# glgerard/MDBN

Measured on AMD Instinct MI355X. Metric: CD-k Gibbs steps/sec (samples/sec), GRBM 4096->1024 CD-1, higher is better.
Workload: dtype f32; 1 GPU; GRBM 4096->1024 CD-1, batch 512 per GPU, fp32, N(0,1) rows resident in HBM (BASELINE configs[1]); global_batch=512, k=1, n_data=32768, parallelism=dp1

## Files before the change

### mdbn_amd/csrc/mdbn_capi.hip

```cpp
#include <hip/hip_runtime.h>
#include "row_pool.h"
#include <dlfcn.h>
#include <algorithm>
#include <atomic>
#include <chrono>
#include <condition_variable>
#include <cstdint>
#include <deque>
#include <initializer_list>
#include <map>
#include <mutex>
#include <set>
#include <thread>
#include <cstdarg>
#include <cstdio>
#include <cstring>
#include <string>
#include <utility>
#include <vector>
#include "mdbn_kernels.h"
#include "mdbn_small.h"
#include "mdbn_thin.h"
#include "mdbn_gchain.h"
#include "mdbn_ais.h"
// ... 754 lines not shown
            EpiArgs e{};
            e.ld = ldh; e.bias = a->hbias; e.mean = keep ? nh : nullptr; e.mean_scale = -1.0f; e.gauss = 0;
            e.sample = (need_sample && keep) ? a->hs : nullptr; e.rng = key((uint32_t)(2 * t));
            e.mean_planes = pb.Pp + B * ldh; e.plane_stride = pb.pp;
            e.sample_plane = need_sample ? pb.hsp : nullptr;
            if (last) { e.colsum = ws.colPneg; e.colsum_kind = 0; }
            if (a->gauss) CHECK(run_affine_planes(ctx, a->comm_cus, pb.Xp + B * ldv, ldv, pb.px, 3, 0, Wp, V, H, Hlive, B, e, false, ws, s, nullptr));
            else CHECK(run_affine_planes(ctx, a->comm_cus, pb.vsp, ldv, B * ldv, 1, 0, Wp, V, H, Hlive, B, e, false, ws, s, nullptr));
            if (a->trace_h && need_sample)
                HIP_OK(hipMemcpyAsync(a->trace_h + (int64_t)t * B * ldh, a->hs, sizeof(float) * B * ldh, hipMemcpyDeviceToDevice, s));
        }
    }
    return MDBN_OK;
}

int planes_statistics(mdbn_ctx* ctx, hipStream_t s, const mdbn_cd_args* a, const Workspace& ws, const PlaneStep& pb, int n_cost,
                      const mdbn_update_args* upd, const mdbn_update_args* defer)
{
    const int64_t B = a->B, V = a->V, Hlive = a->H, ldv = V, ldh = a->ldh, H = ldh;
    const StatsView st(a->stats, V, ldv, ldh);
    const Plan sp = plan_stats(V, H, 2 * B, ldh, false);
    PlaneGemmArgs g{};
    g.A = pb.Xp; g.lda = ldv; g.pa = pb.px; g.ap = 3;
    g.B = pb.Pp; g.ldb = ldh; g.pb = pb.pp;
    g.M = (int)V; g.N = (int)H; g.K = (int)(2 * B);
    g.tiles_m = (int)(V / 128); g.tiles_n = (int)(H / 128); g.splitk = sp.splitk; g.kchunk = sp.kchunk;
    g.fin_enabled = 0;
    int bal = sp.splitk == 1 ? bal_blocks(ctx, a->comm_cus, (int64_t)g.tiles_m * g.tiles_n, 2 * B / 32) : 0;
    if (bal && ((int64_t)bal * 2 * 16384 > ws.slab_floats || V * ldh * 4 >= (int64_t)1 << 31)) bal = 0;
    const bool fuse_upd = !bal && upd != nullptr && g_opt_fused_update && sp.splitk == 1;
    auto set_gather_ahead = [&]() {
        if (g.upd.early && g_opt_gather_ahead && a->next_indexes && pb.Xother && !pb.keep) {
            const int nwg = g.tiles_m * g.tiles_n, nt = (int)(2 * B / 32);
            const int rpw = (int)((B + nwg - 1) / nwg), passes = (int)((ldv / 8 + 255) / 256);
            if (rpw * passes <= 4 && 16 / (nt >= 20 ? 1 : 2) + 4 + 1 <= nt - 3) {
                g.ga.src = a->data; g.ga.n_rows = a->n_data; g.ga.ld_src = ldv;
                g.ga.idx = a->next_indexes; g.ga.idx64 = a->index_is_64;
                g.ga.B = (int)B; g.ga.rpw = rpw; g.ga.passes = passes;
                g.ga.P = pb.Xother; g.ga.plane_stride = pb.px; g.ga.ld = ldv;
                if (a->ahead_done) *a->ahead_done = 1;
            }
        }
    };
    if (fuse_upd) {
        BiasUpd bu;
        fill_bias_upd(bu, *upd, Hlive);
        g.fused = 2;
        g.fin_enabled = 1;
        g.fin = make_fin_args(ws.colPpos, ws.colPneg, ws.colV, row_groups(B), ldh, ldv, ws.cost_partials, n_cost, st.s_h, st.s_v,
                              st.cost, &bu);
        fill_upd(g.upd, *upd, V, ldh, pb.Wp);
        g.upd.early = g_opt_early_w && upd->lambda_1 == 0.f && (upd->weightcost == 0.f || upd->W0 != nullptr) &&
                      2 * B / 32 >= 12 && g_opt_planes_mfma == 16 && !g_opt_bf16_inputs;
        set_gather_ahead();
        HIP_OK(timed_gemm_planes(LAY_MN, LAY_MN, g, s));
        return MDBN_OK;
    }
    if (sp.splitk == 1 && g_opt_fused_finalize) {
        g.fin_enabled = 1;
        g.fin = make_fin_args(ws.colPpos, ws.colPneg, ws.colV, row_groups(B), ldh, ldv, ws.cost_partials, n_cost, st.s_h, st.s_v,
                              st.cost, nullptr);
    } else {
        HIP_OK(launch_finalize_stats(ws.colPpos, ws.colPneg, ws.colV, row_groups(B), ldh, ldv, ws.cost_partials, n_cost, st.s_h,
                                     st.s_v, st.cost, nullptr, s));
    }
    g.fused = 0; g.ldc = ldh; g.slab_stride = V * ldh;
    if (defer) {
        const bool splitphase = g_opt_early_w && g_opt_planes_mfma == 16 && !g_opt_bf16_inputs && defer->phase == 3 &&
                                defer->lambda_1 == 0.f && (defer->weightcost == 0.f || defer->W0 != nullptr) &&
                                defer->stats != a->stats;
        const int64_t flat = bal ? (((V * ldh / 4 + bal - 1) / bal + 511) / 512) * 512 : 0;
        const bool inside = splitphase && (bal ? (flat <= 16 * 512 && (int64_t)g.tiles_m * g.tiles_n * (2 * B / 32) / bal >= 20)
                                               : (sp.splitk == 1 && 2 * B / 32 >= 20));
        g.upd.flat_per_wg = flat;
        if (inside) {
            fill_upd(g.upd, *defer, V, ldh, reinterpret_cast<unsigned short*>(defer->W_planes));
            g.upd.l1 = 0.f; g.upd.Sprev = defer->stats; g.upd.early = 2;
            const StatsView prev(const_cast<float*>(defer->stats), V, ldv, ldh);
            DeferredBias& d = g.db;
            d.on = 1; d.hb = defer->hbias; d.hbs = defer->hbias_speed; d.vb = defer->vbias; d.vbs = defer->vbias_speed;
            d.s_h = prev.s_h; d.s_v = prev.s_v; d.cost_sum = prev.cost; d.H = Hlive; d.V = V;
            d.lr = defer->lr; d.mu = defer->momentum; d.inv_rows = 1.0f / defer->n_rows;
            d.cost_scale = defer->cost_scale; d.cost_out = defer->cost_out;
            if (!bal) set_gather_ahead();
        } else {
            HIP_OK(launch_whole_update(*defer, s));
        }
    }
    if (bal) {
        g.xcd_group = 1;
        g.C = st.S; g.bal = bal; g.fused = 4; g.kchunk = (int)(2 * B); g.c_bytes = V * ldh * 4;
        g.scratch = ws.slabs;
        HIP_OK(timed_gemm_planes(LAY_MN, LAY_MN, g, s));
    } else if (sp.splitk == 1) {
        g.C = st.S;
        HIP_OK(timed_gemm_planes(LAY_MN, LAY_MN, g, s));
    } else {
        REQUIRE(sp.slab_floats(V, ldh) <= ws.slab_floats, "internal: statistic slabs exceed workspace");
        g.C = ws.slabs;
        HIP_OK(timed_gemm_planes(LAY_MN, LAY_MN, g, s));
        if (upd && g_opt_fused_update) {
            HIP_OK(launch_update(whole_rule(*upd), s, ws.slabs, sp.splitk, g.slab_stride, pb.Wp));
            return MDBN_OK;
        }
        HIP_OK(launch_sum_slabs(ws.slabs, sp.splitk, g.slab_stride, V * ldh, st.S, s));
    }
// ... 2044 lines not shown
```

### mdbn_amd/csrc/mdbn_kernels.h

```cpp
#pragma once
#include <hip/hip_runtime.h>
#include <stdint.h>
#include "philox.h"
#include "../../include/mdbn_hip.h"

namespace mdbn {

enum { LAY_K = 0, LAY_MN = 1 };

struct EpiArgs {
    const float* slabs;
    int64_t slab_stride;
    int nsplit;
    int rows, cols;
    int64_t ld;
    const float* bias;
    float* pre;
    float* mean;
    float* sample;
    float mean_scale;
    int gauss;
    const float* target;
    int64_t ld_target;
    const void* target_idx;
// ... 50 lines not shown
    const float* A;
    const float* B;
    float* C;
    int64_t lda, ldb, ldc;
    int64_t slab_stride;
    int M, N, K;
    int Nst;
    int kchunk;
    int splitk, tiles_m, tiles_n;
    int bn;
    int bk;
    int inner_m;
    int x6;
    int x6_pw;
    int cw;
    unsigned long long* stamps;
    int skinny;
    int mi;
    int ni;
    int fused;
    EpiArgs epi;
    UpdEpi upd;
    int fin_enabled;
    FinArgs fin;
};



struct GatherAhead {
    const float* src; int64_t n_rows, ld_src;
    const void* idx; int idx64;
    int B, rpw, passes;
    unsigned short* P; int64_t plane_stride, ld;
};

struct PlaneGemmArgs {
    const unsigned short* A; int64_t lda, pa;
    const unsigned short* B; int64_t ldb, pb;
    float* C; int64_t ldc, slab_stride;
    int M, N, K, kchunk, splitk, tiles_m, tiles_n;
    int ap;
    int ms;
    int bn;
    int fused;
    int slab_tail;
    unsigned long long* stamps;
    int bal;
    int xcd_group;
    float* scratch;
    int64_t c_bytes;
    EpiArgs epi;
    UpdEpi upd;
    int fin_enabled;
    FinArgs fin;
    GatherAhead ga;
    DeferredBias db;
};

__host__ __device__ inline int bal_first_unit(int w, int P, int64_t U) { return (int)(((int64_t)w * U) / P); }
__host__ __device__ inline int bal_block_of(int64_t u, int P, int64_t U) { return (int)(((u + 1) * P - 1) / U); }
__host__ __device__ inline int bal_rem_blocks(int tiles, int S, int P)
{
    const int64_t Ur = (int64_t)(tiles - (tiles / P) * P) * S;
    return Ur < P ? (int)Ur : P;
}
__host__ __device__ inline int bal_tile_slabs(int t, int tiles, int S, int P)
{
    const int Tf = (tiles / P) * P;
    if (t < Tf) return 1;
    const int64_t Ur = (int64_t)(tiles - Tf) * S, u0 = (int64_t)(t - Tf) * S;
    const int Pr = bal_rem_blocks(tiles, S, P);
    return bal_block_of(u0 + S - 1, Pr, Ur) - bal_block_of(u0, Pr, Ur) + 1;
}
hipError_t launch_gemm_planes(int la, int lb, const PlaneGemmArgs& g, hipStream_t s);
bool slab_tail_ok(const PlaneGemmArgs& g, int la, int lb);
hipError_t launch_gemm_planes_bal(int la, int lb, const PlaneGemmArgs& g, hipStream_t s);
int bal_max_segments(int tiles, int stages, int P);
int bal_segment_host(int tiles, int S, int P, int w, int k, int* tile, int* s0, int* s1, int* nseg, int* nt);
hipError_t launch_split_planes(const float* X, int64_t rows, int64_t ld, unsigned short* P, int64_t plane_stride, hipStream_t s);
hipError_t launch_gather_planes(const float* src, int64_t n_rows, int64_t cols_ld, int64_t ld_src, const void* idx, int idx64,
                                int64_t n_idx, float* dst, int64_t ld_dst, unsigned short* P, int64_t plane_stride, hipStream_t s);

int epilogue_blocks(int64_t rows, int64_t ld);
int epilogue_cw(int64_t rows, int64_t ld);
void set_epilogue_cw(int cw);
void set_epilogue_threads(int t);
inline int row_groups(int64_t B) { return (int)((B + 3) / 4); }

hipError_t launch_gemm(int la, int lb, const GemmArgs& g, hipStream_t s);
hipError_t launch_act_epilogue(const EpiArgs& e, hipStream_t s);
hipError_t launch_sum_slabs(const float* slabs, int nsplit, int64_t slab_stride, int64_t n,
                            float* out, hipStream_t s);
hipError_t launch_gather_slim(const float* src, int64_t n_rows, int64_t cols_ld, int64_t ld_src, const void* idx, int idx64,
                              int64_t n_idx, float* dst, int64_t ld_dst, int blocks, int threads, hipStream_t s);
hipError_t launch_gather(const float* src, int64_t n_rows, int64_t cols_ld, int64_t ld_src,
                         const void* idx, int idx64, int64_t n_idx, float* dst, int64_t ld_dst,
                         hipStream_t s);
hipError_t launch_colsum_groups(const float* X, const float* Y, int rows, int64_t ld, float* out, hipStream_t s);
FinArgs make_fin_args(const float* posP, const float* negP, const float* partV, int ngroups, int64_t ldh, int64_t ldv,
                      const float* cost_partials, int n_cost, float* s_h, float* s_v, float* cost,
                      const BiasUpd* bias_update);
hipError_t launch_finalize_stats(const float* posP, const float* negP, const float* partV, int ngroups,
                                 int64_t ldh, int64_t ldv, const float* cost_partials, int n_cost,
                                 float* s_h, float* s_v, float* cost, const BiasUpd* bias_update, hipStream_t s);
hipError_t launch_update(const mdbn_update_args& a, hipStream_t s, const float* slabs = nullptr, int nslab = 1,
                         int64_t slab_stride = 0, unsigned short* Wp = nullptr);
hipError_t launch_free_energy(const float* slabs, int nsplit, int64_t slab_stride, int64_t ldh, int H,
                              const float* hbias, const float* x, int64_t ldv, int V, const float* vbias,
                              int gauss, int64_t rows, float* out, hipStream_t s);
hipError_t launch_round_flip(const float* x, float* out, int64_t rows, int64_t cols, int64_t ld, int64_t flip_col, hipStream_t s);
hipError_t launch_pl_cost(const float* fe, const float* fe_flip, int64_t rows, float n_visible, float* out, hipStream_t s);
hipError_t launch_recon_cost(const float* pre, int64_t ldp, const float* tgt, int64_t ldt, int64_t rows, int64_t cols, int gauss,
                             float scale, float* partials, int n_partials, float* out, hipStream_t s);
hipError_t launch_tanh(float* x, int64_t rows, int64_t cols, int64_t ld, hipStream_t s);
hipError_t launch_count_nonfinite(const float* x, int64_t n, int* count, hipStream_t s);
hipError_t launch_narrow_bf16(const float* x, unsigned short* y, int64_t n, hipStream_t s);
hipError_t launch_widen_bf16(const unsigned short* y, float* x, int64_t n, hipStream_t s);
hipError_t launch_rng_fill(float* out, int64_t rows, int64_t cols, int64_t ld, const PhiloxKey& k,
                           int normal, hipStream_t s);

}
```

### mdbn_amd/csrc/mdbn_planes.hip

```cpp
#include <hip/hip_runtime.h>
#include <algorithm>
#include <stdint.h>
#include "mdbn_kernels.h"
#include "mdbn_device.h"

namespace mdbn {

typedef __bf16 pbf16x8 __attribute__((ext_vector_type(8)));
typedef short ps16x4 __attribute__((ext_vector_type(4)));
typedef short ps16x8 __attribute__((ext_vector_type(8)));
typedef float pf32x16 __attribute__((ext_vector_type(16)));
typedef float pf32x4 __attribute__((ext_vector_type(4)));
typedef unsigned int pu32x4b __attribute__((ext_vector_type(4)));

#ifndef PL_ARGS_EARLY
#define PL_ARGS_EARLY 1
#endif
constexpr int PL_PLANE = 8192, PL_STAGE = 6 * PL_PLANE, PL_NSTAGE = 3, PL_LW = 4;

__device__ __forceinline__ void pl_glds16(const void* g, unsigned lds_off, char* smem)
{
    __builtin_amdgcn_global_load_lds((const __attribute__((address_space(1))) void*)g,
                                     (__attribute__((address_space(3))) void*)(smem + lds_off), 16, 0, 0);
}

template <int MS> __device__ __forceinline__ int pl_row_swz(int row)
{
    return MS == 32 ? ((row >> 2) & 3) : ((4 - ((row >> 2) & 3)) & 3);
}
template <int MS> __device__ __forceinline__ int pl_col_swz(int k)
{
    return MS == 32 ? ((k & 3) << 2) : (((k & 3) | (((k >> 3) & 1) << 2)) << 1);
}

#ifdef MDBN_STAMP
#if defined(MDBN_STAMP_NARROW)
#define PL_STAMP_COND (LA == LAY_K && LB == LAY_K && AP == 1 && BN == 64)
#elif defined(MDBN_STAMP_STATS)
#define PL_STAMP_COND (LA == LAY_MN && LB == LAY_MN && AP == 3)
#else
#define PL_STAMP_COND (LA == LAY_K && LB == LAY_MN && AP == 3)
#endif
#define PL_STAMP(SLOT)                                                                        \
    do {                                                                                      \
        if (PL_STAMP_COND && g.stamps && w == 0 && lane == 0)                                 \
            g.stamps[(int64_t)blockIdx.x * 16 + (SLOT)] = wall_clock64();                     \
    } while (0)
#else
#define PL_STAMP(SLOT) do {} while (0)
#endif
struct EarlySpeed { float4 sp[16], w0[16]; };
__device__ __forceinline__ void deferred_bias_update(const DeferredBias& d, int wave, int lane)
{
    for (int64_t i = (int64_t)blockIdx.x * 256 + wave * 64 + lane; i < d.H + d.V; i += (int64_t)gridDim.x * 256) {
        if (i < d.H) {
            const float sn = upd_speed(upd_scale(d.s_h[i], d.inv_rows), d.hbs[i], d.mu);
            d.hbs[i] = sn;
            d.hb[i] = upd_param(d.hb[i], 1.0f, sn, d.lr);
        } else {
            const int64_t j = i - d.H;
            const float sn = upd_speed(upd_scale(d.s_v[j], d.inv_rows), d.vbs[j], d.mu);
            d.vbs[j] = sn;
            d.vb[j] = upd_param(d.vb[j], 1.0f, sn, d.lr);
        }
    }
    if (blockIdx.x == 0 && wave == 0 && lane == 0 && d.cost_out) d.cost_out[0] = d.cost_sum[0] * d.cost_scale;
}

template <int LA, int LB, int AP, int MS, bool EARLYW = false, int BN = 128>
// ... 69 lines not shown
        }
    }
    asm volatile("s_waitcnt vmcnt(0)" ::: "memory");
    PL_STAMP(3);
    __builtin_amdgcn_s_barrier();
    if (nt > 1) { PL_ISSUE(1); }
    if (nt > 2) { PL_ISSUE(2); }
    const int lt = w * 64 + lane;
    int it = 0;
#define LD_SYNC()                                                                             \
    do {                                                                                      \
        if (it + 2 < nt) asm volatile("s_waitcnt vmcnt(%0)" :: "n"(PER) : "memory");          \
        else asm volatile("s_waitcnt vmcnt(0)" ::: "memory");                                 \
        __builtin_amdgcn_s_barrier();                 \
    } while (0)
#define ASM_LOAD4(DST, PTR) asm volatile("global_load_dwordx4 %0, %1, off" : "=v"(DST) : "v"(PTR) : "memory")
#define ASM_WAIT(N) do { asm volatile("s_waitcnt vmcnt(%0)" :: "n"(N) : "memory"); __builtin_amdgcn_sched_barrier(0); } while (0)
    if constexpr (EARLYW) {
        if (g.upd.early == 2) {
            const float decay = upd_decay(g.upd.lr, g.upd.l2);
            const int64_t lane_off = (int64_t)(m0 + (lt >> 5)) * g.upd.ld + n0 + 4 * (lt & 31);
            const bool has_wc = g.upd.wc != 0.0f;
            const float* w0base = has_wc ? g.upd.W0 : g.upd.Ws;
            pf32x4 dw[16], ds[16], dt[16], d0[16];
            ASM_LOAD4(dw[0], g.upd.W + lane_off); ASM_LOAD4(ds[0], g.upd.Ws + lane_off);
            ASM_LOAD4(dt[0], g.upd.Sprev + lane_off); ASM_LOAD4(d0[0], w0base + lane_off);
#pragma unroll
            for (int i = 0; i < 16; ++i) {
                LD_SYNC();
                if (i + 1 < 16) {
                    const int64_t o1 = lane_off + (int64_t)8 * (i + 1) * g.upd.ld;
                    ASM_LOAD4(dw[i + 1], g.upd.W + o1); ASM_LOAD4(ds[i + 1], g.upd.Ws + o1);
                    ASM_LOAD4(dt[i + 1], g.upd.Sprev + o1); ASM_LOAD4(d0[i + 1], w0base + o1);
                }
                PL_ISSUE(it + 3);
                if (i + 1 < 16) ASM_WAIT(PER + 4); else ASM_WAIT(PER);
                const int64_t off = lane_off + (int64_t)8 * i * g.upd.ld;
                float4 sn, wn;
#pragma unroll
                for (int j = 0; j < 4; ++j) {
                    const float w0j = has_wc ? d0[i][j] : 0.0f;
                    const float snj = upd_speed(upd_grad(dt[i][j], g.upd.inv_bs, g.upd.wc, w0j), ds[i][j], g.upd.mu);
                    setc(sn, j, snj);
                    setc(wn, j, upd_param(dw[i][j], decay, snj, g.upd.lr));
                }
                *reinterpret_cast<float4*>(g.upd.Ws + off) = sn;
                *reinterpret_cast<float4*>(g.upd.W + off) = wn;
                if (g.upd.Wp) store_planes4(g.upd.Wp, g.upd.wp_stride, off, wn);
                ++it;
            }
        } else if (g.upd.early) {
            const float decay = upd_decay(g.upd.lr, g.upd.l2);
            const int64_t lane_off = (int64_t)(m0 + (lt >> 5)) * g.upd.ld + n0 + 4 * (lt & 31);
#define CW_STORE(WV, SV, CH)                                                                  \
    do {                                                                                      \
        const int64_t off_ = lane_off + (int64_t)8 * (CH) * g.upd.ld;                         \
        const float4 w4_ = make_float4(WV[0], WV[1], WV[2], WV[3]), s4_ = make_float4(SV[0], SV[1], SV[2], SV[3]); \
        float4 wn_;                                                                           \
        _Pragma("unroll") for (int j_ = 0; j_ < 4; ++j_) setc(wn_, j_, upd_param(comp(w4_, j_), decay, comp(s4_, j_), g.upd.lr)); \
        *reinterpret_cast<float4*>(g.upd.W + off_) = wn_;                                     \
        if (g.upd.Wp) store_planes4(g.upd.Wp, g.upd.wp_stride, off_, wn_);                    \
    } while (0)
            if (nt >= 20) {
                pf32x4 cw[17], cs[17];
                ASM_LOAD4(cw[0], g.upd.W + lane_off); ASM_LOAD4(cs[0], g.upd.Ws + lane_off);
#pragma unroll
                for (int i = 0; i < 16; ++i) {
                    LD_SYNC();
                    if (i + 1 < 16) {
                        ASM_LOAD4(cw[i + 1], g.upd.W + lane_off + (int64_t)8 * (i + 1) * g.upd.ld);
                        ASM_LOAD4(cs[i + 1], g.upd.Ws + lane_off + (int64_t)8 * (i + 1) * g.upd.ld);
                    }
                    PL_ISSUE(it + 3);
                    if (i + 1 < 16) ASM_WAIT(PER + 2); else ASM_WAIT(PER);
                    CW_STORE(cw[i], cs[i], i);
                    es->sp[i] = make_float4(cs[i][0], cs[i][1], cs[i][2], cs[i][3]);
                    ++it;
                }
            } else {
                pf32x4 cw[18], cs[18];
                ASM_LOAD4(cw[0], g.upd.W + lane_off); ASM_LOAD4(cs[0], g.upd.Ws + lane_off);
                ASM_LOAD4(cw[1], g.upd.W + lane_off + (int64_t)8 * g.upd.ld); ASM_LOAD4(cs[1], g.upd.Ws + lane_off + (int64_t)8 * g.upd.ld);
#pragma unroll
                for (int i = 0; i < 8; ++i) {
                    LD_SYNC();
                    if (i + 1 < 8) {
                        ASM_LOAD4(cw[2 * i + 2], g.upd.W + lane_off + (int64_t)8 * (2 * i + 2) * g.upd.ld);
                        ASM_LOAD4(cs[2 * i + 2], g.upd.Ws + lane_off + (int64_t)8 * (2 * i + 2) * g.upd.ld);
                        ASM_LOAD4(cw[2 * i + 3], g.upd.W + lane_off + (int64_t)8 * (2 * i + 3) * g.upd.ld);
                        ASM_LOAD4(cs[2 * i + 3], g.upd.Ws + lane_off + (int64_t)8 * (2 * i + 3) * g.upd.ld);
                    }
                    PL_ISSUE(it + 3);
                    if (i + 1 < 8) ASM_WAIT(PER + 4); else ASM_WAIT(PER);
                    CW_STORE(cw[2 * i], cs[2 * i], 2 * i);
                    CW_STORE(cw[2 * i + 1], cs[2 * i + 1], 2 * i + 1);
                    es->sp[2 * i] = make_float4(cs[2 * i][0], cs[2 * i][1], cs[2 * i][2], cs[2 * i][3]);
                    es->sp[2 * i + 1] = make_float4(cs[2 * i + 1][0], cs[2 * i + 1][1], cs[2 * i + 1][2], cs[2 * i + 1][3]);
                    ++it;
                }
            }
#undef CW_STORE
        }
        if (g.upd.early) {
            if (g.ga.idx) {
                const int64_t (&srow)[4] = ga_srow;
                const int64_t ld8 = g.ga.ld >> 3;
                const int nunits = g.ga.rpw * g.ga.passes;
                pf32x4 ga[4], gb[4];
#define GU_ADDR(U)                                                                            \
    const int i_r0 = (U) / g.ga.passes, pass_ = (U) - i_r0 * g.ga.passes, i_r = i_r0 < 4 ? i_r0 : 3;   \
    const int64_t c_ = (int64_t)pass_ * 256 + lt, cc_ = c_ < ld8 ? c_ : ld8 - 1;              \
    const int64_t sr_ = i_r == 0 ? srow[0] : i_r == 1 ? srow[1] : i_r == 2 ? srow[2] : srow[3]; \
    const float* p_ = g.ga.src + sr_ * g.ga.ld_src + 8 * cc_;
#define GU_LOAD(K, U) do { GU_ADDR(U) ASM_LOAD4(ga[K], p_); ASM_LOAD4(gb[K], p_ + 4); } while (0)
#define GU_APPLY(K, U)                                                                        \
    do {                                                                                      \
        const int i_r = (U) / g.ga.passes, pass_ = (U) - i_r * g.ga.passes;                   \
        const int r_ = (int)blockIdx.x * g.ga.rpw + i_r;                                      \
        const int64_t c_ = (int64_t)pass_ * 256 + lt;                                         \
        if ((U) < nunits && r_ < g.ga.B && c_ < ld8) {                                        \
            const float v_[8] = {ga[K][0], ga[K][1], ga[K][2], ga[K][3], gb[K][0], gb[K][1], gb[K][2], gb[K][3]}; \
            unsigned short q_[3][8];                                                          \
            _Pragma("unroll") for (int j_ = 0; j_ < 8; ++j_) split3(v_[j_], q_[0][j_], q_[1][j_], q_[2][j_]); \
            _Pragma("unroll") for (int p_ = 0; p_ < 3; ++p_) {                                \
                uint4 wv_;                                                                    \
                wv_.x = q_[p_][0] | ((unsigned)q_[p_][1] << 16); wv_.y = q_[p_][2] | ((unsigned)q_[p_][3] << 16); \
                wv_.z = q_[p_][4] | ((unsigned)q_[p_][5] << 16); wv_.w = q_[p_][6] | ((unsigned)q_[p_][7] << 16); \
                *reinterpret_cast<uint4*>(g.ga.P + p_ * g.ga.plane_stride + (int64_t)r_ * g.ga.ld + 8 * c_) = wv_; \
            }                                                                                 \
        }                                                                                     \
    } while (0)
                LD_SYNC(); GU_LOAD(0, 0); PL_ISSUE(it + 3); ++it;
#define GU_SLOT(K)                                                                            \
    do {                                                                                      \
        LD_SYNC();                                                                            \
        if ((K) < 3) { GU_LOAD((K) + 1, (K) + 1); }                                           \
        PL_ISSUE(it + 3);                                                                     \
        if ((K) < 3) ASM_WAIT(PER + 2); else ASM_WAIT(PER);                                   \
        GU_APPLY(K, K); ++it;                                                                 \
    } while (0)
                GU_SLOT(0); GU_SLOT(1); GU_SLOT(2); GU_SLOT(3);
#undef GU_SLOT
#undef GU_LOAD
#undef GU_APPLY
#undef GU_ADDR
            }
        }
    }
    for (; it < nt; ++it) {
        LD_SYNC();
        if (it + 3 < nt) { PL_ISSUE(it + 3); }
    }
#undef ASM_LOAD4
#undef ASM_WAIT
#undef LD_SYNC
    if constexpr (EARLYW) {
        if (g.upd.early == 1) {
#pragma unroll
            for (int j = 0; j < 16; ++j) {
                const int64_t off = (int64_t)(m0 + 8 * j + (lt >> 5)) * g.upd.ld + n0 + 4 * (lt & 31);
                es->w0[j] = g.upd.W0 ? *reinterpret_cast<const float4*>(g.upd.W0 + off) : make_float4(0.f, 0.f, 0.f, 0.f);
            }
        }
    }
    PL_STAMP(4);
#undef PL_ISSUE
}

template <int LAY>
__device__ __forceinline__ pbf16x8 pl_frag(const char* plane, int off0, int off1)
{
    if constexpr (LAY == LAY_K) {
        return *reinterpret_cast<const pbf16x8*>(plane + off0);
    } else {
        const ps16x4 lo = __builtin_amdgcn_ds_read_tr16_b64_v4i16((__attribute__((address_space(3))) ps16x4*)(plane + off0));
        const ps16x4 hi = __builtin_amdgcn_ds_read_tr16_b64_v4i16((__attribute__((address_space(3))) ps16x4*)(plane + off1));
        const ps16x8 v = {lo[0], lo[1], lo[2], lo[3], hi[0], hi[1], hi[2], hi[3]};
        return __builtin_bit_cast(pbf16x8, v);
    }
}
// ... 422 lines not shown
                const int lt = (wave - 4) * 64 + lane;
                constexpr int LDT = 128 + 8;
#pragma unroll
                for (int j = 0; j < 16; ++j) {
                    const int row = 8 * j + (lt >> 5), c4 = lt & 31;
                    const float4 st = *reinterpret_cast<const float4*>(T + row * LDT + 4 * c4);
                    float4 sn;
#pragma unroll
                    for (int c = 0; c < 4; ++c)
                        setc(sn, c, upd_speed(upd_grad(comp(st, c), g.upd.inv_bs, g.upd.wc, comp(es.w0[j], c)), comp(es.sp[j], c), g.upd.mu));
                    *reinterpret_cast<float4*>(g.upd.Ws + (int64_t)(m0 + row) * g.upd.ld + n0 + 4 * c4) = sn;
                }
            }
        }
        else fused_update_epilogue<128, 128, NT>(g.upd, T, m0, n0);
#ifdef MDBN_STAMP
        if (PL_STAMP_COND && g.stamps && threadIdx.x == 0) {
            asm volatile("s_waitcnt vmcnt(0)" ::: "memory");
            g.stamps[(int64_t)blockIdx.x * 16 + 12] = wall_clock64();
        }
#endif
    }
}

template <int LA, int LB, int AP, int FUSED, int MS, int BN = 128>
static hipError_t launch_planes_m(const PlaneGemmArgs& g, hipStream_t s)
{
    auto kern = gemm_planes_kernel<LA, LB, AP, FUSED, MS, BN>;
    static bool attr_set = false;
    constexpr int lds = PL_NSTAGE * PL_STAGE;
    if (!attr_set) {
        hipError_t e = hipFuncSetAttribute(reinterpret_cast<const void*>(kern), hipFuncAttributeMaxDynamicSharedMemorySize, lds);
        if (e != hipSuccess) return e;
        attr_set = true;
    }
    hipLaunchKernelGGL(kern, dim3(g.tiles_m * g.tiles_n * g.splitk), dim3(64 * (4 + PL_LW)), lds, s, g);
    return hipGetLastError();
}

template <int LA, int LB, int AP, int FUSED>
static hipError_t launch_planes_t(const PlaneGemmArgs& g, hipStream_t s)
{
    if constexpr (AP == 0) return launch_planes_m<LA, LB, 0, FUSED, 16>(g, s);
    else return g.ms == 32 ? launch_planes_m<LA, LB, AP, FUSED, 32>(g, s) : launch_planes_m<LA, LB, AP, FUSED, 16>(g, s);
}

#ifndef PL_TAIL_T
#define PL_TAIL_T 2
#endif
#ifndef PL_TAIL_WT
#define PL_TAIL_WT 1
#endif
struct PlSlabOut {
    __amdgpu_buffer_rsrc_t rsrc;
    int lane_off, ldc4;
};

template <int LA, int LB, int AP, int TC, int PAR, int WT>
__device__ __forceinline__ void pl_tail16(const char* smem, int nb, const int (&offA)[4][2], const int (&offB)[4][2],
                                          pf32x4a (&acc)[4][4], pbf16x8 (&A0)[3][2], pbf16x8 (&B0)[3][2], pbf16x8 (&A1)[3][2],
                                          pbf16x8 (&B1)[3][2], const PlSlabOut& so)
{
    constexpr int NBH = 2;
    PL_CONSUME_CONSTS_SW(true);
    int sb[TC];
#pragma unroll
    for (int s = 0; s < TC; ++s) sb[s] = ((nb + s) % PL_NSTAGE) * PL_STAGE;
#define PL_TAIL_ITEM(I, CA, CB, NXA, NXB)                                                     \
    do {                                                                                      \
        const int q_ = (I) / TC, s_ = (I) % TC, q1_ = ((I) + 1) / TC, s1_ = ((I) + 1) % TC;   \
        const int ah_ = q_ >> 1, bh_ = (((q_ + 1) >> 1) & 1) ^ PAR;                           \
        const int ah1_ = q1_ >> 1, bh1_ = (((q1_ + 1) >> 1) & 1) ^ PAR;                       \
        if (q_ == 0) PL_RAW_BARRIER();             \
         \
                               \
        int o1_ = sb[s1_];                                                                    \
        asm volatile("" : "+s"(o1_));                                                         \
        if ((I) + 1 < 4 * TC) { RD_A(NXA, smem + o1_, ah1_); RD_B(NXB, smem + o1_, bh1_); }   \
        MMQ(CA, CB, ah_, bh_);                                                                \
        if ((I) + 1 < 4 * TC) { ORD(RA + RB); }                                               \
        if (s_ == TC - 1) {                        \
            _Pragma("unroll") for (int a = 0; a < 2; ++a)                                     \
                _Pragma("unroll") for (int b = 0; b < 2; ++b) {                               \
                    const pu32x4b v_ = __builtin_bit_cast(pu32x4b, acc[2 * ah_ + a][2 * bh_ + b]); \
                    const int off_ = 16 * (2 * ah_ + a) * so.ldc4 + 64 * (2 * bh_ + b);       \
                    if (WT == 2 || (WT == 1 && q_ < 3)) __builtin_amdgcn_raw_buffer_store_b128(v_, so.rsrc, so.lane_off, off_, 16); \
                    else __builtin_amdgcn_raw_buffer_store_b128(v_, so.rsrc, so.lane_off, off_, 0); \
                }                                                                             \
        }                                                                                     \
        __builtin_amdgcn_sched_barrier(0);         \
    } while (0)
#pragma unroll
    for (int j = 0; j < 2 * TC; ++j) {
        PL_TAIL_ITEM(2 * j, A0, B0, A1, B1);
        PL_TAIL_ITEM(2 * j + 1, A1, B1, A0, B0);
    }
#undef PL_TAIL_ITEM
}

template <int LA, int LB, int AP, int T, int WT>
__device__ __forceinline__ void pl_consume16_tail(char* smem, int nt, int lane, int wm, int wn, pf32x4a (&acc)[4][4], const PlSlabOut& so)
{
    static_assert(T >= 1 && T <= PL_NSTAGE, "the tail stages must all be resident in the ring");
    long long bar_wait = 0;
    (void)bar_wait;
    constexpr int NBH = 2;
    int offA[4][2], offB[4][2];
    pl_offsets16<LA, LB>(lane, wm, wn, offA, offB);
    PL_CONSUME_CONSTS_SW(true);
    pbf16x8 Alo[3][2], Ahi[3][2], Blo[3][2], Bhi[3][2];
    const int tc = nt < T ? 1 : T, nb = nt - tc;
    RD_A(Alo, smem, 0);
    RD_B(Blo, smem, 0);
    for (int it = 0; it < nb; it += 2) {
        {
            const char* base = smem + (it % PL_NSTAGE) * PL_STAGE;
            const char* next = smem + ((it + 1) % PL_NSTAGE) * PL_STAGE;
            PL_STAGE_EVEN(base, next, PL_MAIN_BARRIER());
        }
        if (it + 1 < nb) {
            const char* base = smem + ((it + 1) % PL_NSTAGE) * PL_STAGE;
            const char* next = smem + ((it + 2) % PL_NSTAGE) * PL_STAGE;
            PL_STAGE_ODD(base, next, PL_MAIN_BARRIER());
        }
    }
    if (tc == T) {
        if (nb & 1) pl_tail16<LA, LB, AP, T, 1, WT>(smem, nb, offA, offB, acc, Alo, Bhi, Ahi, Blo, so);
        else pl_tail16<LA, LB, AP, T, 0, WT>(smem, nb, offA, offB, acc, Alo, Blo, Ahi, Bhi, so);
    } else if constexpr (T > 1) {
        if (nb & 1) pl_tail16<LA, LB, AP, 1, 1, WT>(smem, nb, offA, offB, acc, Alo, Bhi, Ahi, Blo, so);
        else pl_tail16<LA, LB, AP, 1, 0, WT>(smem, nb, offA, offB, acc, Alo, Blo, Ahi, Bhi, so);
    }
}

template <int AP, int T, int WT>
__global__ __launch_bounds__(64 * (4 + PL_LW)) void gemm_planes_slabtail_kernel(PlaneGemmArgs g)
{
    extern __shared__ __attribute__((aligned(16))) char smem[];
#if PL_ARGS_EARLY
    asm volatile("" :: "s"(g.A), "s"(g.lda), "s"(g.pa), "s"(g.B), "s"(g.ldb), "s"(g.pb), "s"(g.C), "s"(g.ldc), "s"(g.slab_stride),
                 "s"(g.kchunk), "s"(g.tiles_m), "s"(g.tiles_n), "s"((int)gridDim.x));
#endif
    const int nwg = gridDim.x, bid = blockIdx.x;
    const int xcd = bid & 7, slot = bid >> 3;
    const int qq = nwg >> 3, rem = nwg & 7;
    const int w = (xcd < rem ? xcd * (qq + 1) : rem * (qq + 1) + (xcd - rem) * qq) + slot;
    const int tiles = g.tiles_m * g.tiles_n;
    const int ks = w / tiles, t = w - ks * tiles;
    int tm, tn;
    if (g.tiles_m <= g.tiles_n) { tn = t / g.tiles_m; tm = t - tn * g.tiles_m; }
    else { tm = t / g.tiles_n; tn = t - tm * g.tiles_n; }
    const int m0 = tm * 128, n0 = tn * 128;
    const int kbeg = ks * g.kchunk;
    const int nt = g.kchunk / 32;
    const int wave = __builtin_amdgcn_readfirstlane(threadIdx.x >> 6);
    const int lane = threadIdx.x & 63;
    if (wave >= 4) {
        pl_loader<LAY_K, LAY_MN, AP, 16, false, 128>(g, smem, wave - 4, lane, m0, n0, kbeg, nt);
        return;
    }
    const int wm = (wave >> 1) * 64, wn = (wave & 1) * 64;
    pf32x4a acc[4][4];
#pragma unroll
    for (int a = 0; a < 4; ++a)
#pragma unroll
        for (int b = 0; b < 4; ++b) acc[a][b] = pf32x4a{0.f, 0.f, 0.f, 0.f};
    PlSlabOut so;
    so.ldc4 = (int)g.ldc * 4;
    so.rsrc = __builtin_amdgcn_make_buffer_rsrc(g.C + (int64_t)ks * g.slab_stride, 0, g.M * so.ldc4, 0x00020000);
    so.lane_off = (m0 + wm + (lane & 15)) * so.ldc4 + (n0 + wn + 4 * (lane >> 4)) * 4;
    __syncthreads();
    pl_consume16_tail<LAY_K, LAY_MN, AP, T, WT>(smem, nt, lane, wm, wn, acc, so);
}

template <int AP>
static hipError_t launch_planes_slabtail(const PlaneGemmArgs& g, hipStream_t s)
{
    auto kern = gemm_planes_slabtail_kernel<AP, PL_TAIL_T, PL_TAIL_WT>;
    static bool attr_set = false;
    constexpr int lds = PL_NSTAGE * PL_STAGE;
    if (!attr_set) {
        hipError_t e = hipFuncSetAttribute(reinterpret_cast<const void*>(kern), hipFuncAttributeMaxDynamicSharedMemorySize, lds);
        if (e != hipSuccess) return e;
        attr_set = true;
    }
    hipLaunchKernelGGL(kern, dim3(g.tiles_m * g.tiles_n * g.splitk), dim3(64 * (4 + PL_LW)), lds, s, g);
    return hipGetLastError();
}

bool slab_tail_ok(const PlaneGemmArgs& g, int la, int lb)
{
    return la == LAY_K && lb == LAY_MN && (g.ap == 1 || g.ap == 3) && g.fused == 0 && g.ms == 16 && g.bn != 64 && !g.bal &&
           (g.ldc & 3) == 0 && (g.slab_stride & 3) == 0 && (reinterpret_cast<uintptr_t>(g.C) & 15) == 0 &&
           (int64_t)g.M * g.ldc * 4 < ((int64_t)1 << 31);
}

hipError_t launch_gemm_planes(int la, int lb, const PlaneGemmArgs& g, hipStream_t s)
{
    if (g.bn == 64) {
        if (g.M % 128 || g.N % 64 || g.K % 32 || g.kchunk != g.K || g.splitk != 1 || g.tiles_m != g.M / 128 || g.tiles_n != g.N / 64 ||
            (g.lda & 7) || (g.ldb & 7) || g.fused != 1 || la != LAY_K || lb != LAY_K || g.ms != 16 || (g.ap != 1 && g.ap != 3))
            return hipErrorInvalidValue;
        return g.ap == 1 ? launch_planes_m<LAY_K, LAY_K, 1, 1, 16, 64>(g, s) : launch_planes_m<LAY_K, LAY_K, 3, 1, 16, 64>(g, s);
    }
    if (g.M % 128 || g.N % 128 || g.kchunk % 32 || g.kchunk * g.splitk != g.K || g.tiles_m != g.M / 128 ||
        g.tiles_n != g.N / 128 || (g.lda & 7) || (g.ldb & 7) || ((g.fused == 1 || g.fused == 2) && g.splitk != 1) ||
        (g.ap != 0 && g.ap != 1 && g.ap != 3))
        return hipErrorInvalidValue;
    if (g.slab_tail) {
        if (!slab_tail_ok(g, la, lb)) return hipErrorInvalidValue;
        return g.ap == 1 ? launch_planes_slabtail<1>(g, s) : launch_planes_slabtail<3>(g, s);
    }
#define PL_CASE(LAV, LBV, APV, FV) \
    if (la == LAV && lb == LBV && g.ap == APV && g.fused == FV) return launch_planes_t<LAV, LBV, APV, FV>(g, s)
    PL_CASE(LAY_K, LAY_MN, 3, 0); PL_CASE(LAY_K, LAY_MN, 3, 1); PL_CASE(LAY_K, LAY_MN, 1, 0); PL_CASE(LAY_K, LAY_MN, 1, 1);
    PL_CASE(LAY_K, LAY_K, 3, 0); PL_CASE(LAY_K, LAY_K, 3, 1); PL_CASE(LAY_K, LAY_K, 1, 0); PL_CASE(LAY_K, LAY_K, 1, 1);
    PL_CASE(LAY_MN, LAY_MN, 3, 0); PL_CASE(LAY_MN, LAY_MN, 3, 2);
    PL_CASE(LAY_K, LAY_MN, 0, 0); PL_CASE(LAY_K, LAY_MN, 0, 1); PL_CASE(LAY_K, LAY_K, 0, 0); PL_CASE(LAY_K, LAY_K, 0, 1);
    PL_CASE(LAY_MN, LAY_MN, 0, 0); PL_CASE(LAY_MN, LAY_MN, 0, 2);
#undef PL_CASE
    return hipErrorInvalidValue;
}

struct BalRange {
    int F, Tf;
    int tA, sA, tB, eB, nrem;
    int pre, nseg, nt;
};
__host__ __device__ inline BalRange bal_range(int w, int P, int tiles, int S)
{
    BalRange r;
    r.F = tiles / P; r.Tf = r.F * P;
    const int64_t Ur = (int64_t)(tiles - r.Tf) * S;
    const int Pr = bal_rem_blocks(tiles, S, P);
    const int u0 = w < Pr ? bal_first_unit(w, Pr, Ur) : 0, u1 = w < Pr ? bal_first_unit(w + 1, Pr, Ur) : 0;
    r.tA = r.sA = r.tB = r.eB = r.nrem = r.pre = 0;
    if (u1 > u0) {
        r.tA = u0 / S; r.sA = u0 - r.tA * S;
        r.tB = (u1 - 1) / S; r.eB = u1 - r.tB * S;
        r.nrem = r.tB - r.tA + 1;
        r.pre = r.nrem == 2 ? 1 : (r.eB != S ? 1 : 0);
    }
    r.nseg = r.F + r.nrem;
    r.nt = r.F * S + (u1 - u0);
    return r;
}
__host__ __device__ inline void bal_segment(const BalRange& r, int w, int k, int S, int& tile, int& s0, int& s1)
{
    if (k < r.pre) {
        if (r.nrem == 2) { tile = r.Tf + r.tB; s0 = 0; s1 = r.eB; }
        else { tile = r.Tf + r.tA; s0 = r.sA; s1 = r.eB; }
    } else if (k < r.pre + r.F) {
        tile = w * r.F + (k - r.pre); s0 = 0; s1 = S;
    } else {
        tile = r.Tf + r.tA; s0 = r.sA; s1 = S;
    }
}

template <int LA, int LB, int AP>
__device__ __forceinline__ void pl_loader_bal(const PlaneGemmArgs& g, char* smem, int w, int lane, int wg, const BalRange& r, int nt, int S)
{
    constexpr int NA = AP == 3 ? 3 : 1, NB = AP == 0 ? 1 : 3;
    constexpr int NQ = 8 * (NA + NB), PER = NQ / PL_LW, PERA = 8 * NA / PL_LW;
    const char* base[PER];
// ... 397 lines not shown
```

Baseline: 3.919 million samples/s.

## Add stats-tail GEMM kernel that parks accumulators in LDS for loader-wave weight update

Adds a specialised fused-update GEMM kernel for the weight-gradient pass. The MFMA waves park their final accumulator halves in freed ring slots of LDS, and the loader waves compute and store the momentum speed update from there. This hands the epilogue work to otherwise idle loader waves and overlaps it with the tail of the GEMM. It also adds an optional buffer-store side-write path for the W, plane and gather stores, which is disabled by default. The new path is gated on slab_tail and early-update conditions, with an extra barrier and an LDS handover that add synchronisation risk.

Measured after the change: 3.968 million samples/s, median of 6. 1.01x the previous value.

```diff
diff --git a/mdbn_amd/csrc/mdbn_capi.hip b/mdbn_amd/csrc/mdbn_capi.hip
--- a/mdbn_amd/csrc/mdbn_capi.hip
+++ b/mdbn_amd/csrc/mdbn_capi.hip
@@ -830,6 +830,7 @@
         fill_upd(g.upd, *upd, V, ldh, pb.Wp);
         g.upd.early = g_opt_early_w && upd->lambda_1 == 0.f && (upd->weightcost == 0.f || upd->W0 != nullptr) &&
                       2 * B / 32 >= 12 && g_opt_planes_mfma == 16 && !g_opt_bf16_inputs;
+        g.stats_tail = g_opt_slab_tail && g.upd.early == 1 && ldh < ((int64_t)1 << 21);
         set_gather_ahead();
         HIP_OK(timed_gemm_planes(LAY_MN, LAY_MN, g, s));
         return MDBN_OK;
diff --git a/mdbn_amd/csrc/mdbn_kernels.h b/mdbn_amd/csrc/mdbn_kernels.h
--- a/mdbn_amd/csrc/mdbn_kernels.h
+++ b/mdbn_amd/csrc/mdbn_kernels.h
@@ -126,6 +126,7 @@
     EpiArgs epi;
     UpdEpi upd;
     int fin_enabled;
+    int stats_tail;
     FinArgs fin;
     GatherAhead ga;
     DeferredBias db;
@@ -148,6 +149,7 @@
 }
 hipError_t launch_gemm_planes(int la, int lb, const PlaneGemmArgs& g, hipStream_t s);
 bool slab_tail_ok(const PlaneGemmArgs& g, int la, int lb);
+bool stats_tail_ok(const PlaneGemmArgs& g, int la, int lb);
 hipError_t launch_gemm_planes_bal(int la, int lb, const PlaneGemmArgs& g, hipStream_t s);
 int bal_max_segments(int tiles, int stages, int P);
 int bal_segment_host(int tiles, int S, int P, int w, int k, int* tile, int* s0, int* s1, int* nseg, int* nt);
diff --git a/mdbn_amd/csrc/mdbn_planes.hip b/mdbn_amd/csrc/mdbn_planes.hip
--- a/mdbn_amd/csrc/mdbn_planes.hip
+++ b/mdbn_amd/csrc/mdbn_planes.hip
@@ -12,9 +12,13 @@
 typedef float pf32x16 __attribute__((ext_vector_type(16)));
 typedef float pf32x4 __attribute__((ext_vector_type(4)));
 typedef unsigned int pu32x4b __attribute__((ext_vector_type(4)));
+typedef unsigned int pu32x2b __attribute__((ext_vector_type(2)));
 
 #ifndef PL_ARGS_EARLY
 #define PL_ARGS_EARLY 1
+#endif
+#ifndef PL_SIDE_WT
+#define PL_SIDE_WT 0
 #endif
 constexpr int PL_PLANE = 8192, PL_STAGE = 6 * PL_PLANE, PL_NSTAGE = 3, PL_LW = 4;
 
@@ -190,14 +194,35 @@
         } else if (g.upd.early) {
             const float decay = upd_decay(g.upd.lr, g.upd.l2);
             const int64_t lane_off = (int64_t)(m0 + (lt >> 5)) * g.upd.ld + n0 + 4 * (lt & 31);
+            const int64_t tile_off = (int64_t)m0 * g.upd.ld + n0;
+            const int tile_elems = 127 * (int)g.upd.ld + 128;
+            const __amdgpu_buffer_rsrc_t side_w = __builtin_amdgcn_make_buffer_rsrc(g.upd.W + tile_off, 0, tile_elems * 4, 0x00020000);
+            __amdgpu_buffer_rsrc_t side_p[3];
+#pragma unroll
+            for (int p = 0; p < 3; ++p)
+                side_p[p] = __builtin_amdgcn_make_buffer_rsrc(g.upd.Wp + p * g.upd.wp_stride + tile_off, 0, g.upd.Wp ? tile_elems * 2 : 0, 0x00020000);
+            (void)side_w; (void)side_p;
 #define CW_STORE(WV, SV, CH)                                                                  \
     do {                                                                                      \
         const int64_t off_ = lane_off + (int64_t)8 * (CH) * g.upd.ld;                         \
         const float4 w4_ = make_float4(WV[0], WV[1], WV[2], WV[3]), s4_ = make_float4(SV[0], SV[1], SV[2], SV[3]); \
         float4 wn_;                                                                           \
         _Pragma("unroll") for (int j_ = 0; j_ < 4; ++j_) setc(wn_, j_, upd_param(comp(w4_, j_), decay, comp(s4_, j_), g.upd.lr)); \
-        *reinterpret_cast<float4*>(g.upd.W + off_) = wn_;                                     \
-        if (g.upd.Wp) store_planes4(g.upd.Wp, g.upd.wp_stride, off_, wn_);                    \
+        if (PL_SIDE_WT) {                                                                     \
+            const int o_ = (int)(off_ - tile_off) * 4;                                        \
+            __builtin_amdgcn_raw_buffer_store_b128(__builtin_bit_cast(pu32x4b, wn_), side_w, o_, 0, 16); \
+            if (g.upd.Wp) {                                                                   \
+                unsigned short q_[3][4];                                                      \
+                _Pragma("unroll") for (int j_ = 0; j_ < 4; ++j_) split3(comp(wn_, j_), q_[0][j_], q_[1][j_], q_[2][j_]); \
+                _Pragma("unroll") for (int p_ = 0; p_ < 3; ++p_) {                            \
+                    const pu32x2b v_ = {q_[p_][0] | ((unsigned)q_[p_][1] << 16), q_[p_][2] | ((unsigned)q_[p_][3] << 16)}; \
+                    __builtin_amdgcn_raw_buffer_store_b64(v_, side_p[p_], o_ >> 1, 0, 16);    \
+                }                                                                             \
+            }                                                                                 \
+        } else {                                                                              \
+            *reinterpret_cast<float4*>(g.upd.W + off_) = wn_;                                 \
+            if (g.upd.Wp) store_planes4(g.upd.Wp, g.upd.wp_stride, off_, wn_);                \
+        }                                                                                     \
     } while (0)
             if (nt >= 20) {
                 pf32x4 cw[17], cs[17];
@@ -245,6 +270,11 @@
                 const int64_t ld8 = g.ga.ld >> 3;
                 const int nunits = g.ga.rpw * g.ga.passes;
                 pf32x4 ga[4], gb[4];
+                __amdgpu_buffer_rsrc_t side_g[3];
+#pragma unroll
+                for (int p = 0; p < 3; ++p)
+                    side_g[p] = __builtin_amdgcn_make_buffer_rsrc(g.ga.P + p * g.ga.plane_stride, 0, g.ga.B * (int)g.ga.ld * 2, 0x00020000);
+                (void)side_g;
 #define GU_ADDR(U)                                                                            \
     const int i_r0 = (U) / g.ga.passes, pass_ = (U) - i_r0 * g.ga.passes, i_r = i_r0 < 4 ? i_r0 : 3;   \
     const int64_t c_ = (int64_t)pass_ * 256 + lt, cc_ = c_ < ld8 ? c_ : ld8 - 1;              \
@@ -264,6 +294,9 @@
                 uint4 wv_;                                                                    \
                 wv_.x = q_[p_][0] | ((unsigned)q_[p_][1] << 16); wv_.y = q_[p_][2] | ((unsigned)q_[p_][3] << 16); \
                 wv_.z = q_[p_][4] | ((unsigned)q_[p_][5] << 16); wv_.w = q_[p_][6] | ((unsigned)q_[p_][7] << 16); \
+                if (PL_SIDE_WT)                                                               \
+                    __builtin_amdgcn_raw_buffer_store_b128(__builtin_bit_cast(pu32x4b, wv_), side_g[p_], (r_ * (int)g.ga.ld + 8 * (int)c_) * 2, 0, 16); \
+                else                                                                          \
                 *reinterpret_cast<uint4*>(g.ga.P + p_ * g.ga.plane_stride + (int64_t)r_ * g.ga.ld + 8 * c_) = wv_; \
             }                                                                                 \
         }                                                                                     \
@@ -792,14 +825,28 @@
 #define PL_TAIL_WT 1
 #endif
 struct PlSlabOut {
+    static constexpr bool HANDOVER = false;
     __amdgpu_buffer_rsrc_t rsrc;
     int lane_off, ldc4;
+    template <int WT>
+    __device__ __forceinline__ void final_quarter(char*, int q, int ah, int bh, const pf32x4a (&acc)[4][4]) const
+    {
+#pragma unroll
+        for (int a = 0; a < 2; ++a)
+#pragma unroll
+            for (int b = 0; b < 2; ++b) {
+                const pu32x4b v = __builtin_bit_cast(pu32x4b, acc[2 * ah + a][2 * bh + b]);
+                const int off = 16 * (2 * ah + a) * ldc4 + 64 * (2 * bh + b);
+                if (WT == 2 || (WT == 1 && q < 3)) __builtin_amdgcn_raw_buffer_store_b128(v, rsrc, lane_off, off, 16);
+                else __builtin_amdgcn_raw_buffer_store_b128(v, rsrc, lane_off, off, 0);
+            }
+    }
 };
 
-template <int LA, int LB, int AP, int TC, int PAR, int WT>
+template <int LA, int LB, int AP, int TC, int PAR, int WT, class OUT>
 __device__ __forceinline__ void pl_tail16(const char* smem, int nb, const int (&offA)[4][2], const int (&offB)[4][2],
                                           pf32x4a (&acc)[4][4], pbf16x8 (&A0)[3][2], pbf16x8 (&B0)[3][2], pbf16x8 (&A1)[3][2],
-                                          pbf16x8 (&B1)[3][2], const PlSlabOut& so)
+                                          pbf16x8 (&B1)[3][2], const OUT& so)
 {
     constexpr int NBH = 2;
     PL_CONSUME_CONSTS_SW(true);
@@ -812,6 +859,10 @@
         const int ah_ = q_ >> 1, bh_ = (((q_ + 1) >> 1) & 1) ^ PAR;                           \
         const int ah1_ = q1_ >> 1, bh1_ = (((q1_ + 1) >> 1) & 1) ^ PAR;                       \
         if (q_ == 0) PL_RAW_BARRIER();             \
+        if (OUT::HANDOVER && (I) == 4 * TC - 1) {  \
+            PIN(CA, NA); PINB(CB, NB);                                                        \
+            PL_RAW_BARRIER();                                                                 \
+        }                                                                                     \
          \
                                \
         int o1_ = sb[s1_];                                                                    \
@@ -819,15 +870,7 @@
         if ((I) + 1 < 4 * TC) { RD_A(NXA, smem + o1_, ah1_); RD_B(NXB, smem + o1_, bh1_); }   \
         MMQ(CA, CB, ah_, bh_);                                                                \
         if ((I) + 1 < 4 * TC) { ORD(RA + RB); }                                               \
-        if (s_ == TC - 1) {                        \
-            _Pragma("unroll") for (int a = 0; a < 2; ++a)                                     \
-                _Pragma("unroll") for (int b = 0; b < 2; ++b) {                               \
-                    const pu32x4b v_ = __builtin_bit_cast(pu32x4b, acc[2 * ah_ + a][2 * bh_ + b]); \
-                    const int off_ = 16 * (2 * ah_ + a) * so.ldc4 + 64 * (2 * bh_ + b);       \
-                    if (WT == 2 || (WT == 1 && q_ < 3)) __builtin_amdgcn_raw_buffer_store_b128(v_, so.rsrc, so.lane_off, off_, 16); \
-                    else __builtin_amdgcn_raw_buffer_store_b128(v_, so.rsrc, so.lane_off, off_, 0); \
-                }                                                                             \
-        }                                                                                     \
+        if (s_ == TC - 1) so.template final_quarter<WT>(const_cast<char*>(smem), q_, ah_, bh_, acc);    \
         __builtin_amdgcn_sched_barrier(0);         \
     } while (0)
 #pragma unroll
@@ -838,8 +881,8 @@
 #undef PL_TAIL_ITEM
 }
 
-template <int LA, int LB, int AP, int T, int WT>
-__device__ __forceinline__ void pl_consume16_tail(char* smem, int nt, int lane, int wm, int wn, pf32x4a (&acc)[4][4], const PlSlabOut& so)
+template <int LA, int LB, int AP, int T, int WT, bool EVEN = false, class OUT>
+__device__ __forceinline__ void pl_consume16_tail(char* smem, int nt, int lane, int wm, int wn, pf32x4a (&acc)[4][4], const OUT& so)
 {
     static_assert(T >= 1 && T <= PL_NSTAGE, "the tail stages must all be resident in the ring");
     long long bar_wait = 0;
@@ -849,7 +892,7 @@
     pl_offsets16<LA, LB>(lane, wm, wn, offA, offB);
     PL_CONSUME_CONSTS_SW(true);
     pbf16x8 Alo[3][2], Ahi[3][2], Blo[3][2], Bhi[3][2];
-    const int tc = nt < T ? 1 : T, nb = nt - tc;
+    const int tc = (EVEN || nt >= T) ? T : 1, nb = nt - tc;
     RD_A(Alo, smem, 0);
     RD_B(Blo, smem, 0);
     for (int it = 0; it < nb; it += 2) {
@@ -864,7 +907,9 @@
             PL_STAGE_ODD(base, next, PL_MAIN_BARRIER());
         }
     }
-    if (tc == T) {
+    if constexpr (EVEN) {
+        pl_tail16<LA, LB, AP, T, 0, WT>(smem, nb, offA, offB, acc, Alo, Blo, Ahi, Bhi, so);
+    } else if (tc == T) {
         if (nb & 1) pl_tail16<LA, LB, AP, T, 1, WT>(smem, nb, offA, offB, acc, Alo, Bhi, Ahi, Blo, so);
         else pl_tail16<LA, LB, AP, T, 0, WT>(smem, nb, offA, offB, acc, Alo, Blo, Ahi, Bhi, so);
     } else if constexpr (T > 1) {
@@ -928,6 +973,131 @@
     return hipGetLastError();
 }
 
+#ifndef PL_STATS_TAIL
+#define PL_STATS_TAIL 1
+#endif
+#ifndef PL_STATS_TAIL_WT
+#define PL_STATS_TAIL_WT 2
+#endif
+constexpr int PL_HALF_LDT = 128 + 8;
+static_assert(64 * PL_HALF_LDT * 4 <= PL_STAGE, "a parked half tile must fit one ring slot");
+
+struct PlStatsPark {
+    static constexpr bool HANDOVER = true;
+    int off0, off1;
+    __device__ __forceinline__ void park(char* base, int ah, int bh, const pf32x4a (&acc)[4][4]) const
+    {
+#pragma unroll
+        for (int a = 0; a < 2; ++a)
+#pragma unroll
+            for (int b = 0; b < 2; ++b)
+                *reinterpret_cast<pf32x4a*>(base + (16 * a * PL_HALF_LDT + 32 * bh + 16 * b) * 4) = acc[2 * ah + a][2 * bh + b];
+    }
+    template <int WT>
+    __device__ __forceinline__ void final_quarter(char* smem, int q, int ah, int bh, const pf32x4a (&acc)[4][4]) const
+    {
+        if (ah == 0) park(smem + off0, 0, bh, acc);
+        if (q == 1) PL_RAW_BARRIER();
+        if (q == 3) {
+            park(smem + off1, 1, 1, acc);
+            park(smem + off1, 1, 0, acc);
+            PL_RAW_BARRIER();
+        }
+    }
+};
+
+template <int HALF, int AUX>
+__device__ __forceinline__ void pl_stats_speed_half(const UpdEpi& u, const char* half, int lt, const EarlySpeed& es,
+                                                    __amdgpu_buffer_rsrc_t rsrc)
+{
+#pragma unroll
+    for (int jj = 0; jj < 8; ++jj) {
+        const int j = 4 * HALF + (jj & 3) + 8 * (jj >> 2);
+        const int row = 8 * j + (lt >> 5), c4 = lt & 31;
+        const int lr = (row & 31) + 32 * (row >> 6);
+        const float4 st = *reinterpret_cast<const float4*>(half + (lr * PL_HALF_LDT + 4 * c4) * 4);
+        pf32x4 sn;
+#pragma unroll
+        for (int c = 0; c < 4; ++c)
+            sn[c] = upd_speed(upd_grad(comp(st, c), u.inv_bs, u.wc, comp(es.w0[j], c)), comp(es.sp[j], c), u.mu);
+        __builtin_amdgcn_raw_buffer_store_b128(__builtin_bit_cast(pu32x4b, sn), rsrc, (row * (int)u.ld + 4 * c4) * 4, 0, AUX);
+    }
+}
+
+template <int WT>
+__global__ __launch_bounds__(64 * (4 + PL_LW)) void gemm_planes_statstail_kernel(PlaneGemmArgs g)
+{
+    extern __shared__ __attribute__((aligned(16))) char smem[];
+#if PL_ARGS_EARLY
+    asm volatile("" :: "s"(g.A), "s"(g.lda), "s"(g.pa), "s"(g.B), "s"(g.ldb), "s"(g.pb), "s"(g.kchunk), "s"(g.tiles_m),
+                 "s"(g.tiles_n), "s"((int)gridDim.x));
+#endif
+    const int nwg = gridDim.x, bid = blockIdx.x;
+    const int xcd = bid & 7, slot = bid >> 3;
+    const int qq = nwg >> 3, rem = nwg & 7;
+    const int t = (xcd < rem ? xcd * (qq + 1) : rem * (qq + 1) + (xcd - rem) * qq) + slot;
+    int tm, tn;
+    if (g.tiles_m <= g.tiles_n) { tn = t / g.tiles_m; tm = t - tn * g.tiles_m; }
+    else { tm = t / g.tiles_n; tn = t - tm * g.tiles_n; }
+    const int m0 = tm * 128, n0 = tn * 128;
+    const int nt = g.kchunk / 32;
+    const int wave = __builtin_amdgcn_readfirstlane(threadIdx.x >> 6);
+    const int lane = threadIdx.x & 63;
+    const int half0 = (nt % PL_NSTAGE) * PL_STAGE, half1 = ((nt + 1) % PL_NSTAGE) * PL_STAGE;
+    if (wave >= 4) {
+        EarlySpeed es;
+        pl_loader<LAY_MN, LAY_MN, 3, 16, true, 128>(g, smem, wave - 4, lane, m0, n0, 0, nt, &es);
+        const int lt = (wave - 4) * 64 + lane;
+        const __amdgpu_buffer_rsrc_t rsrc = __builtin_amdgcn_make_buffer_rsrc(
+            g.upd.Ws + (int64_t)m0 * g.upd.ld + n0, 0, (127 * (int)g.upd.ld + 128) * 4, 0x00020000);
+        asm volatile("s_barrier" ::: "memory");
+        pl_stats_speed_half<0, (WT != 0 ? 16 : 0)>(g.upd, smem + half0, lt, es, rsrc);
+        asm volatile("s_barrier" ::: "memory");
+        asm volatile("s_barrier" ::: "memory");
+        pl_stats_speed_half<1, (WT == 2 ? 16 : 0)>(g.upd, smem + half1, lt, es, rsrc);
+        return;
+    }
+    if (g.fin_enabled) {
+        const int nu = fin_units(g.fin);
+        for (int unit = wave * (int)gridDim.x + (int)blockIdx.x; unit <= nu; unit += 4 * (int)gridDim.x)
+            finalize_unit(g.fin, unit, lane);
+    }
+    const int wm = (wave >> 1) * 64, wn = (wave & 1) * 64;
+    pf32x4a acc[4][4];
+#pragma unroll
+    for (int a = 0; a < 4; ++a)
+#pragma unroll
+        for (int b = 0; b < 4; ++b) acc[a][b] = pf32x4a{0.f, 0.f, 0.f, 0.f};
+    PlStatsPark pk;
+    const int lane_share = (((wm >> 6) * 32 + (lane & 15)) * PL_HALF_LDT + wn + 4 * (lane >> 4)) * 4;
+    pk.off0 = half0 + lane_share;
+    pk.off1 = half1 + lane_share;
+    __syncthreads();
+    pl_consume16_tail<LAY_MN, LAY_MN, 3, 2, 0, true>(smem, nt, lane, wm, wn, acc, pk);
+}
+
+[[maybe_unused]] static hipError_t launch_planes_statstail(const PlaneGemmArgs& g, hipStream_t s)
+{
+    auto kern = gemm_planes_statstail_kernel<PL_STATS_TAIL_WT>;
+    static bool attr_set = false;
+    constexpr int lds = PL_NSTAGE * PL_STAGE;
+    if (!attr_set) {
+        hipError_t e = hipFuncSetAttribute(reinterpret_cast<const void*>(kern), hipFuncAttributeMaxDynamicSharedMemorySize, lds);
+        if (e != hipSuccess) return e;
+        attr_set = true;
+    }
+    hipLaunchKernelGGL(kern, dim3(g.tiles_m * g.tiles_n), dim3(64 * (4 + PL_LW)), lds, s, g);
+    return hipGetLastError();
+}
+
+bool stats_tail_ok(const PlaneGemmArgs& g, int la, int lb)
+{
+    const int nt = g.kchunk / 32;
+    return la == LAY_MN && lb == LAY_MN && g.ap == 3 && g.fused == 2 && g.upd.early == 1 && g.ms == 16 && g.bn != 64 && !g.bal &&
+           g.splitk == 1 && nt >= 12 && (nt & 1) == 0 && (g.upd.ld & 3) == 0 && g.upd.ld < ((int64_t)1 << 21) &&
+           (reinterpret_cast<uintptr_t>(g.upd.Ws) & 15) == 0;
+}
+
 bool slab_tail_ok(const PlaneGemmArgs& g, int la, int lb)
 {
     return la == LAY_K && lb == LAY_MN && (g.ap == 1 || g.ap == 3) && g.fused == 0 && g.ms == 16 && g.bn != 64 && !g.bal &&
@@ -950,6 +1120,12 @@
     if (g.slab_tail) {
         if (!slab_tail_ok(g, la, lb)) return hipErrorInvalidValue;
         return g.ap == 1 ? launch_planes_slabtail<1>(g, s) : launch_planes_slabtail<3>(g, s);
+    }
+    if (g.stats_tail) {
+        if (!stats_tail_ok(g, la, lb)) return hipErrorInvalidValue;
+#if PL_STATS_TAIL
+        return launch_planes_statstail(g, s);
+#endif
     }
 #define PL_CASE(LAV, LBV, APV, FV) \
     if (la == LAV && lb == LBV && g.ap == APV && g.fused == FV) return launch_planes_t<LAV, LBV, APV, FV>(g, s)
```
